# wamuumu/query-recommendation-system

Measured on AMD Instinct MI355X. Metric: MinHash signatures/sec through the whole hot path (signatures -> LSH candidates -> pair scoring -> top-K), higher is better.
Workload: dtype u16/int32 MinHash values, uint64 keys and pairs (integer); float64 cosine

## Files before the change

query-recommendation-system_amd/csrc/pairs.hip:

```cpp
#include "common.h"

constexpr int PAIR_THREADS = 256;
constexpr int PAIR_IPT = 4;
constexpr int PAIR_TILE = PAIR_THREADS * PAIR_IPT;

constexpr int CMP_THREADS = 256;
constexpr int CMP_IPT = 8;
constexpr int CMP_TILE = CMP_THREADS * CMP_IPT;

constexpr int PAIR_HALO = 128;

__device__ static inline uint32_t mix_hi(uint64_t k, int hsh) { return (uint32_t)(qr_mix64(k) >> hsh); }

__device__ static inline void stage_tile(const uint64_t *__restrict__ k, int64_t nq, int64_t tile_start, int hsh,
                                         uint64_t *sk, uint32_t *sh) {
  for (int idx = threadIdx.x; idx < PAIR_HALO + PAIR_TILE; idx += PAIR_THREADS) {
    const int64_t g = tile_start - PAIR_HALO + idx;
    uint64_t key = 0;
    if (g >= 0 && g < nq) key = k[g];
    sk[idx] = key;
    sh[idx] = mix_hi(key, hsh);
  }
}

// ... 845 lines not shown

QRLSH_EXPORT size_t qrlsh_region_unique_workspace_bytes(int64_t nids, int32_t group_bits) {
  if (nids <= 0 || group_bits < 0 || group_bits > 8) return 64;
  const int64_t nr = region_count(nids, group_bits);
  return (size_t)(4 * (nr + 1) + ceil_div64(nr + 1, SCANL_CHUNK) + 2) * sizeof(uint64_t);
}

__global__ __launch_bounds__(256) void region_spans_kernel(const uint32_t *__restrict__ counts, int64_t nr, uint32_t cap,
                                                           uint64_t *__restrict__ starts, uint64_t *__restrict__ ends,
                                                           const uint32_t *__restrict__ scatter_ovf,
                                                           uint64_t *__restrict__ ovf_out) {
  const int64_t r = (int64_t)blockIdx.x * blockDim.x + threadIdx.x;
  if (r == 0 && ovf_out) *ovf_out = *scatter_ovf;
  if (r > nr) return;
  starts[r] = (uint64_t)r * cap;
  ends[r] = (uint64_t)r * cap + (r < nr ? min(counts[r], cap) : 0u);
}

template <typename W = uint64_t>
static int region_unique_count_impl(const char *name, const W *grouped, int64_t n, const uint32_t *regions_counts,
                                    uint32_t cap, int32_t group_bits, int32_t id_bits, int64_t nids, uint64_t *tmp,
                                    void *workspace, size_t workspace_bytes, uint64_t *total_overflow_out, void *stream,
                                    const uint32_t *scatter_ovf = nullptr) {
  QR_CHECK_ARG(n >= 0 && total_overflow_out && nids > 0 && nids <= (1ll << 32), "%s: bad arguments", name);
  QR_CHECK_ARG(group_bits >= 0 && group_bits <= 8 && id_bits >= 1 && id_bits <= 31 && nids <= (1ll << id_bits) &&
                   (group_bits + id_bits < 32 || (group_bits + id_bits == 32 && nids < (1ll << id_bits))),
               "%s: group_bits=%d / id_bits=%d (need group_bits <= 8, id_bits <= 31, group_bits + id_bits <= 32)", name,
               group_bits, id_bits);
  hipStream_t st = static_cast<hipStream_t>(stream);
  if (hipMemsetAsync(total_overflow_out, 0, (scatter_ovf ? 3 : 2) * sizeof(uint64_t), st) != hipSuccess) {
    qrlsh_set_error("%s: hipMemsetAsync failed", name);
    return QRLSH_EHIP;
  }
  if (n == 0) return QRLSH_OK;
  QR_CHECK_ARG(grouped && tmp && workspace, "%s: null pointer", name);
  if (workspace_bytes < qrlsh_region_unique_workspace_bytes(nids, group_bits)) {
    qrlsh_set_error("%s: workspace %zu < %zu bytes", name, workspace_bytes,
                    qrlsh_region_unique_workspace_bytes(nids, group_bits));
    return QRLSH_EWORKSPACE;
  }
  const int64_t nr = region_count(nids, group_bits);
  QR_CHECK_ARG(nr <= 2147483647ll, "%s: too many regions", name);
  uint64_t *starts = static_cast<uint64_t *>(workspace), *counts = starts + (nr + 1), *biglist = counts + (nr + 1);
  uint64_t *nbig = biglist + nr, *sums = nbig + 1;
  uint64_t *ends = sums + ceil_div64(nr + 1, SCANL_CHUNK) + 1;
  if (hipMemsetAsync(counts + nr, 0, sizeof(uint64_t), st) != hipSuccess ||
      hipMemsetAsync(nbig, 0, sizeof(uint64_t), st) != hipSuccess) {
    qrlsh_set_error("%s: hipMemsetAsync failed", name);
    return QRLSH_EHIP;
  }
  if (regions_counts) {
    QR_LAUNCH("region_bounds", region_spans_kernel, dim3((unsigned)ceil_div64(nr + 1, 256)), dim3(256), 0, st, regions_counts,
              nr, cap, starts, ends, scatter_ovf, scatter_ovf ? total_overflow_out + 2 : nullptr);
  } else {
    if constexpr (sizeof(W) == 8) {
      QR_LAUNCH("region_bounds", region_bounds_kernel, dim3((unsigned)ceil_div64(nr + 1, 256)), dim3(256), 0, st, grouped, n,
                32 + group_bits, nr, starts);
    }
    ends = starts + 1;
  }
  QR_LAUNCH("region_unique", region_unique_kernel<W>, dim3((unsigned)nr), dim3(RG_THREADS), 0, st, grouped,
            (const uint64_t *)starts, (const uint64_t *)ends, tmp, counts, biglist,
            reinterpret_cast<unsigned long long *>(nbig), group_bits, id_bits);
  QR_LAUNCH("region_unique_big", region_unique_big_kernel<W>, dim3((unsigned)(nr < RG_BIG_GRID ? nr : RG_BIG_GRID)),
            dim3(RG_THREADS), 0, st, grouped, (const uint64_t *)starts, (const uint64_t *)ends, tmp, counts,
            (const uint64_t *)biglist, (const unsigned long long *)nbig, total_overflow_out + 1, group_bits, id_bits);
  qr_scan_u64(counts, nr + 1, total_overflow_out, sums, st);
  QR_LAUNCH_CHECK(name);
  return QRLSH_OK;
}

QRLSH_EXPORT int qrlsh_region_unique_count(const uint64_t *grouped, int64_t n, int32_t group_bits, int32_t id_bits,
                                           int64_t nids, uint64_t *tmp, void *workspace, size_t workspace_bytes,
                                           uint64_t *total_overflow_out, void *stream) {
  return region_unique_count_impl("qrlsh_region_unique_count", grouped, n, nullptr, 0u, group_bits, id_bits, nids, tmp,
                                  workspace, workspace_bytes, total_overflow_out, stream);
}

QRLSH_EXPORT int qrlsh_region_unique_count_regions(const uint64_t *regions, const uint32_t *counts, int64_t cap, int64_t n,
                                                   int32_t group_bits, int32_t id_bits, int64_t nids, uint64_t *tmp,
                                                   void *workspace, size_t workspace_bytes, uint64_t *total_overflow_out,
                                                   void *stream) {
  QR_CHECK_ARG(counts && cap > 0 && cap < (1ll << 32), "qrlsh_region_unique_count_regions: bad arguments");
  return region_unique_count_impl("qrlsh_region_unique_count_regions", regions, n, counts, (uint32_t)cap, group_bits, id_bits,
                                  nids, tmp, workspace, workspace_bytes, total_overflow_out, stream);
}

QRLSH_EXPORT int qrlsh_region_unique_count_regions3(const uint64_t *regions, const uint32_t *counts, int64_t cap, int64_t n,
                                                    int32_t group_bits, int32_t id_bits, int64_t nids, uint64_t *tmp,
                                                    void *workspace, size_t workspace_bytes, const uint32_t *scatter_overflow,
                                                    uint64_t *out3, void *stream) {
  QR_CHECK_ARG(counts && scatter_overflow && cap > 0 && cap < (1ll << 32), "qrlsh_region_unique_count_regions3: bad arguments");
  return region_unique_count_impl("qrlsh_region_unique_count_regions3", regions, n, counts, (uint32_t)cap, group_bits, id_bits,
                                  nids, tmp, workspace, workspace_bytes, out3, stream, scatter_overflow);
}

QRLSH_EXPORT int qrlsh_region_unique_count_regions32(const uint32_t *regions, const uint32_t *counts, int64_t cap, int64_t n,
                                                     int32_t group_bits, int32_t id_bits, int64_t nids, uint64_t *tmp,
                                                     void *workspace, size_t workspace_bytes,
                                                     const uint32_t *scatter_overflow, uint64_t *out3, void *stream) {
  QR_CHECK_ARG(counts && scatter_overflow && cap > 0 && cap < (1ll << 32), "qrlsh_region_unique_count_regions32: bad arguments");
  return region_unique_count_impl<uint32_t>("qrlsh_region_unique_count_regions32", regions, n, counts, (uint32_t)cap, group_bits,
                                            id_bits, nids, tmp, workspace, workspace_bytes, out3, stream, scatter_overflow);
}

QRLSH_EXPORT int qrlsh_region_unique_fill(const uint64_t *tmp, int64_t n, int32_t group_bits, int64_t nids,
                                          const void *workspace, uint64_t *out, void *stream) {
  QR_CHECK_ARG(n >= 0 && nids > 0 && group_bits >= 0 && group_bits <= 8, "qrlsh_region_unique_fill: bad arguments");
  if (n == 0) return QRLSH_OK;
  QR_CHECK_ARG(tmp && workspace && out, "qrlsh_region_unique_fill: null pointer");
  const int64_t nr = region_count(nids, group_bits);
  const uint64_t *starts = static_cast<const uint64_t *>(workspace), *offs = starts + (nr + 1);
  QR_LAUNCH("region_gather", region_gather_kernel, dim3((unsigned)nr), dim3(256), 0, static_cast<hipStream_t>(stream), tmp,
            offs, starts, out);
  QR_LAUNCH_CHECK("qrlsh_region_unique_fill");
  return QRLSH_OK;
}

QRLSH_EXPORT int qrlsh_topk_count(const uint64_t *sorted_edges, int64_t n_edges, int32_t K, int32_t id_bits,
                                  void *workspace, size_t workspace_bytes, uint64_t *total_out, void *stream) {
  QR_CHECK_ARG(K > 0 && id_bits >= 0 && id_bits <= 32, "qrlsh_topk_count: bad K=%d or id_bits=%d (need <= 32)", K,
               id_bits);
  return compact_count<PRED_TOPK>(sorted_edges, n_edges, K, id_bits + 11, workspace, workspace_bytes, total_out, stream,
                                  "qrlsh_topk_count");
}

QRLSH_EXPORT int qrlsh_topk_fill(const uint64_t *sorted_edges, const uint32_t *sorted_dst, int64_t n_edges, int32_t K,
                                 int32_t id_bits, const void *workspace, int32_t *src_out, int32_t *dst_out,
                                 int32_t *milli_out, void *stream) {
  return qrlsh_topk_fill_based(sorted_edges, sorted_dst, n_edges, K, id_bits, 0, workspace, src_out, dst_out, milli_out,
                               stream);
}

QRLSH_EXPORT int qrlsh_topk_fill_based(const uint64_t *sorted_edges, const uint32_t *sorted_dst, int64_t n_edges,
                                       int32_t K, int32_t id_bits, int64_t src_base, const void *workspace,
                                       int32_t *src_out, int32_t *dst_out, int32_t *milli_out, void *stream) {
  QR_CHECK_ARG(K > 0 && id_bits >= 0 && id_bits <= 32 && n_edges >= 0 && src_base >= 0 && src_base < (1ll << 31),
               "qrlsh_topk_fill: bad arguments");
  QR_CHECK_ARG((id_bits == 0) == (sorted_dst != nullptr), "qrlsh_topk_fill: sorted_dst goes with id_bits == 0");
  if (n_edges == 0) return QRLSH_OK;
  QR_CHECK_ARG(sorted_edges && workspace && src_out && dst_out && milli_out, "qrlsh_topk_fill: null pointer");
  QR_LAUNCH("topk_fill", (compact_fill_kernel<PRED_TOPK>), dim3((unsigned)ceil_div64(n_edges, CMP_TILE)),
                     dim3(CMP_THREADS), 0, static_cast<hipStream_t>(stream), sorted_edges, n_edges, K, id_bits + 11,
                     id_bits, sorted_dst, static_cast<const uint64_t *>(workspace), nullptr, src_out, dst_out, milli_out,
                     (int32_t)src_base);
  QR_LAUNCH_CHECK("qrlsh_topk_fill");
  return QRLSH_OK;
}

__device__ static inline uint32_t rev_src(uint64_t w, int id_bits, bool wide) {
  return (uint32_t)(wide ? w >> 11 : w >> (id_bits + 11));
}

constexpr uint32_t SEL_UNSET = 0xFFFFFFFFu;
constexpr int SEL_GAP = 32;
constexpr int EB_RUN = 4;
__device__ static inline int64_t edge_src(const uint64_t *__restrict__ a, int64_t t, bool fwd, int id_bits, bool wide) {
  return (int64_t)(fwd ? (uint32_t)(a[t] >> 32) : rev_src(a[t], id_bits, wide));
}
__global__ __launch_bounds__(256) void edge_bounds_kernel(const uint64_t *__restrict__ pairs,
                                                          const uint64_t *__restrict__ rev, int64_t n, int64_t nq,
                                                          int id_bits, int wide, uint32_t *__restrict__ fstart,
                                                          uint32_t *__restrict__ rstart, int y0 = 0) {
  const bool fwd = blockIdx.y + y0 == 0;
  const uint64_t *a = fwd ? pairs : rev;
  uint32_t *start = fwd ? fstart : rstart;
  const bool w = wide != 0;
  const int64_t t0 = ((int64_t)blockIdx.x * blockDim.x + threadIdx.x) * EB_RUN;
  uint64_t x[EB_RUN];
  if (t0 + EB_RUN <= n && ((uintptr_t)a & 15) == 0) {
    const ulonglong2 *v = reinterpret_cast<const ulonglong2 *>(a + t0);
#pragma unroll
    for (int k = 0; k < EB_RUN; k += 2) {
      const ulonglong2 u = v[k >> 1];
      x[k] = u.x;
      x[k + 1] = u.y;
    }
  } else {
#pragma unroll
    for (int k = 0; k < EB_RUN; ++k) x[k] = t0 + k < n ? a[t0 + k] : 0ull;
  }
  int64_t s[EB_RUN];
#pragma unroll
  for (int k = 0; k < EB_RUN; ++k)
    s[k] = t0 + k < n ? (int64_t)(fwd ? (uint32_t)(x[k] >> 32) : rev_src(x[k], id_bits, w)) : nq;
  int64_t p = __shfl_up(s[EB_RUN - 1], 1, WAVE);
  if ((threadIdx.x & (WAVE - 1)) == 0) p = t0 > 0 && t0 <= n ? edge_src(a, t0 - 1, fwd, id_bits, w) : -1;
#pragma unroll
  for (int k = 0; k < EB_RUN; ++k) {
    const int64_t t = t0 + k;
    if (t > n) break;
    if (s[k] - p > SEL_GAP) {
      if (s[k] <= nq) start[s[k]] = (uint32_t)t;
    } else {
      for (int64_t q = p + 1; q <= s[k] && q <= nq; ++q) start[q] = (uint32_t)t;
    }
    p = s[k];
  }
}

__global__ __launch_bounds__(256) void edge_bounds_fix_kernel(const uint64_t *__restrict__ pairs,
                                                              const uint64_t *__restrict__ rev, int64_t n, int64_t nq,
                                                              int id_bits, int wide, uint32_t *__restrict__ fstart,
                                                              uint32_t *__restrict__ rstart, int y0 = 0) {
  const bool fwd = blockIdx.y + y0 == 0;
  const uint64_t *a = fwd ? pairs : rev;
  uint32_t *start = fwd ? fstart : rstart;
  const int64_t q = (int64_t)blockIdx.x * blockDim.x + threadIdx.x;
  if (q > nq || start[q] != SEL_UNSET) return;
  int64_t lo = 0, hi = n;
  while (lo < hi) {
    const int64_t mid = (lo + hi) >> 1;
    if (edge_src(a, mid, fwd, id_bits, wide != 0) >= q) hi = mid;
    else lo = mid + 1;
  }
  start[q] = (uint32_t)lo;
}

constexpr int SEL_SHORT = 16;
constexpr int SEL_LONG = 64;
constexpr int SEL_MAXK = 256;
constexpr int SEL_LIST_GRID = 1024;

constexpr int LEN_QPB = 4096;
__global__ __launch_bounds__(256) void topk_len_kernel(const uint32_t *__restrict__ fstart,
                                                       const uint32_t *__restrict__ rstart, int64_t nq, int K,
                                                       uint64_t *__restrict__ cnt, uint32_t *__restrict__ medlist,
                                                       uint32_t *__restrict__ longlist,
                                                       unsigned long long *__restrict__ nlists,
                                                       uint64_t *__restrict__ wgsum) {
  __shared__ uint32_t smed[LEN_QPB], slng[LEN_QPB], sval[LEN_QPB + LEN_QPB / 16];
  __shared__ uint64_t sscan[4];
  __shared__ uint32_t nmed, nlng;
  __shared__ unsigned long long bmed, blng;
  const int lane = threadIdx.x & (WAVE - 1);
  const uint64_t lt_mask = (1ull << lane) - 1ull;
  auto lpad = [](int i) { return i + (i >> 4); };
  if (threadIdx.x == 0) {
    nmed = 0;
    nlng = 0;
  }
  __syncthreads();
  const int64_t q0 = (int64_t)blockIdx.x * LEN_QPB;
#pragma unroll 4
  for (int it = 0; it < LEN_QPB / 256; ++it) {
    const int64_t q = q0 + it * 256 + threadIdx.x;
    uint64_t c = 0;
    if (q < nq) c = (uint64_t)(fstart[q + 1] - fstart[q]) + (rstart[q + 1] - rstart[q]);
    sval[lpad(it * 256 + threadIdx.x)] = (uint32_t)(c > (uint64_t)K ? (uint64_t)K : c);
    const bool med = c > (uint64_t)SEL_SHORT && c <= (uint64_t)SEL_LONG, lng = c > (uint64_t)SEL_LONG;
    const uint64_t mm = __ballot(med), ml = __ballot(lng);
    uint32_t pm = 0, pl = 0;
    if (lane == 0) {
      if (mm) pm = atomicAdd(&nmed, (uint32_t)__popcll(mm));
      if (ml) pl = atomicAdd(&nlng, (uint32_t)__popcll(ml));
    }
    pm = __shfl(pm, 0, WAVE);
    pl = __shfl(pl, 0, WAVE);
    if (med) smed[pm + (uint32_t)__popcll(mm & lt_mask)] = (uint32_t)q;
    if (lng) slng[pl + (uint32_t)__popcll(ml & lt_mask)] = (uint32_t)q;
  }
  __syncthreads();
  if (threadIdx.x == 0) {
    bmed = nmed ? __hip_atomic_fetch_add(&nlists[0], (unsigned long long)nmed, __ATOMIC_RELAXED, __HIP_MEMORY_SCOPE_AGENT) : 0ull;
    blng = nlng ? __hip_atomic_fetch_add(&nlists[1], (unsigned long long)nlng, __ATOMIC_RELAXED, __HIP_MEMORY_SCOPE_AGENT) : 0ull;
  }
  __syncthreads();
  for (uint32_t k = threadIdx.x; k < nmed; k += 256) medlist[bmed + k] = smed[k];
  for (uint32_t k = threadIdx.x; k < nlng; k += 256) longlist[blng + k] = slng[k];
  constexpr int PER = LEN_QPB / 256;
  uint32_t v[PER], sum = 0;
#pragma unroll
  for (int k = 0; k < PER; ++k) {
    v[k] = sval[lpad(threadIdx.x * PER + k)];
    sum += v[k];
  }
  uint64_t total;
  uint32_t run = (uint32_t)block_excl_scan_u64_256((uint64_t)sum, sscan, &total);
#pragma unroll
  for (int k = 0; k < PER; ++k) {
    sval[lpad(threadIdx.x * PER + k)] = run;
    run += v[k];
  }
  __syncthreads();
  for (int k = threadIdx.x; k < LEN_QPB; k += 256)
    if (q0 + k <= nq) cnt[q0 + k] = sval[lpad(k)];
  if (threadIdx.x == 0) wgsum[blockIdx.x] = total;
}

__global__ __launch_bounds__(256) void topk_off_add_kernel(uint64_t *__restrict__ off, int64_t m,
                                                           const uint64_t *__restrict__ wgsum) {
  const uint64_t add = wgsum[blockIdx.x];
  const int64_t q0 = (int64_t)blockIdx.x * LEN_QPB;
  if (add == 0) return;
#pragma unroll 4
  for (int k = threadIdx.x; k < LEN_QPB; k += 256)
    if (q0 + k < m) off[q0 + k] += add;
}

__device__ static inline uint64_t sel_key(uint32_t x, uint32_t rs, uint32_t nr, uint32_t fs,
                                          const uint64_t *__restrict__ pairs, const int32_t *__restrict__ milli,
                                          const uint64_t *__restrict__ rev, const uint32_t *__restrict__ rdst,
                                          int id_bits, uint64_t idm) {
  if (x < nr) {
    const uint64_t w = rev[rs + x];
    return rdst ? (w & 0x7FFull) << 32 | rdst[rs + x] : ((w >> id_bits) & 0x7FFull) << 32 | (w & idm);
  }
  const uint32_t y = fs + (x - nr);
  return (uint64_t)(uint32_t)(1000 - milli[y]) << 32 | (uint32_t)pairs[y];
}

template <int S> __device__ static inline uint64_t row_ror64(uint64_t v) {
  const int lo = __builtin_amdgcn_update_dpp(0, (int)(uint32_t)v, 0x120 + S, 0xF, 0xF, false);
  const int hi = __builtin_amdgcn_update_dpp(0, (int)(uint32_t)(v >> 32), 0x120 + S, 0xF, 0xF, false);
  return (uint64_t)(uint32_t)hi << 32 | (uint32_t)lo;
}
template <int S> __device__ static inline uint32_t row_rank(uint64_t mine) {
  uint32_t r = row_ror64<S>(mine) < mine;
  if constexpr (S > 1) r += row_rank<S - 1>(mine);
  return r;
}

constexpr int SEL_QPG = 4;
__global__ __launch_bounds__(256) void topk_select_short_kernel(const uint64_t *__restrict__ pairs,
                                                                const int32_t *__restrict__ milli,
                                                                const uint64_t *__restrict__ rev,
                                                                const uint32_t *__restrict__ rdst,
                                                                const uint32_t *__restrict__ fstart,
                                                                const uint32_t *__restrict__ rstart,
                                                                const uint64_t *__restrict__ off, int64_t nq, int K,
                                                                int id_bits, int32_t *__restrict__ src_out,
                                                                int32_t *__restrict__ dst_out,
                                                                int32_t *__restrict__ milli_out) {
  const int64_t group = ((int64_t)blockIdx.x * blockDim.x + threadIdx.x) >> 4;
  const int64_t ngroups = ((int64_t)gridDim.x * blockDim.x) >> 4;
  const uint32_t l = threadIdx.x & 15;
  const uint64_t idm = id_bits >= 32 ? 0xFFFFFFFFull : (1ull << id_bits) - 1ull;
  uint32_t fs[SEL_QPG], rs[SEL_QPG], nr[SEL_QPG], len[SEL_QPG];
  uint64_t o0[SEL_QPG], mine[SEL_QPG];
#pragma unroll
  for (int c = 0; c < SEL_QPG; ++c) {
    const int64_t q = group + (int64_t)c * ngroups;
    uint32_t nf = 0;
    fs[c] = rs[c] = nr[c] = 0;
    o0[c] = 0;
    if (q < nq) {
      fs[c] = fstart[q];
      nf = fstart[q + 1] - fs[c];
      rs[c] = rstart[q];
      nr[c] = rstart[q + 1] - rs[c];
      o0[c] = off[q];
    }
    len[c] = nf + nr[c];
    if (len[c] > (uint32_t)SEL_SHORT) len[c] = 0;
  }
#pragma unroll
  for (int c = 0; c < SEL_QPG; ++c)
    mine[c] = l < len[c] ? sel_key(l, rs[c], nr[c], fs[c], pairs, milli, rev, rdst, id_bits, idm) : ~0ull;
#pragma unroll
  for (int c = 0; c < SEL_QPG; ++c) {
    const uint32_t rank = row_rank<15>(mine[c]);
    if (l < len[c] && rank < (uint32_t)K) {
      const uint64_t o = o0[c] + rank;
      src_out[o] = (int32_t)(group + (int64_t)c * ngroups);
      dst_out[o] = (int32_t)(uint32_t)mine[c];
      milli_out[o] = 1000 - (int32_t)(uint32_t)(mine[c] >> 32);
    }
  }
}

__global__ __launch_bounds__(256) void topk_select_medium_kernel(const uint64_t *__restrict__ pairs,
                                                                 const int32_t *__restrict__ milli,
                                                                 const uint64_t *__restrict__ rev,
                                                                 const uint32_t *__restrict__ rdst,
                                                                 const uint32_t *__restrict__ fstart,
                                                                 const uint32_t *__restrict__ rstart,
                                                                 const uint64_t *__restrict__ off,
                                                                 const uint32_t *__restrict__ medlist,
                                                                 const unsigned long long *__restrict__ nlists, int K,
                                                                 int id_bits, int32_t *__restrict__ src_out,
                                                                 int32_t *__restrict__ dst_out,
                                                                 int32_t *__restrict__ milli_out) {
  const int lane = threadIdx.x & (WAVE - 1);
  const uint64_t idm = id_bits >= 32 ? 0xFFFFFFFFull : (1ull << id_bits) - 1ull;
  const unsigned long long nm = nlists[0], nwaves = (unsigned long long)gridDim.x * (blockDim.x / WAVE);
  for (unsigned long long e = (unsigned long long)blockIdx.x * (blockDim.x / WAVE) + (threadIdx.x >> 6); e < nm;
       e += nwaves) {
    const uint32_t q = medlist[e];
    const uint32_t fs = fstart[q], nf = fstart[q + 1] - fs, rs = rstart[q], nr = rstart[q + 1] - rs;
    const uint32_t len = nf + nr;
    const uint64_t mine = (uint32_t)lane < len ? sel_key(lane, rs, nr, fs, pairs, milli, rev, rdst, id_bits, idm) : ~0ull;
    uint32_t rank = 0;
#pragma unroll 9
    for (int s = 1; s < WAVE; ++s) {
      const int from = (lane + s) & (WAVE - 1);
      const uint32_t lo = (uint32_t)__shfl((int)(uint32_t)mine, from, WAVE), hi = (uint32_t)__shfl((int)(uint32_t)(mine >> 32), from, WAVE);
      rank += ((uint64_t)hi << 32 | lo) < mine;
    }
    if ((uint32_t)lane < len && rank < (uint32_t)K) {
      const uint64_t o = off[q] + rank;
      src_out[o] = (int32_t)q;
      dst_out[o] = (int32_t)(uint32_t)mine;
      milli_out[o] = 1000 - (int32_t)(uint32_t)(mine >> 32);
    }
  }
}

__global__ __launch_bounds__(256) void topk_select_long_kernel(const uint64_t *__restrict__ pairs,
                                                               const int32_t *__restrict__ milli,
                                                               const uint64_t *__restrict__ rev,
                                                               const uint32_t *__restrict__ rdst,
                                                               const uint32_t *__restrict__ fstart,
                                                               const uint32_t *__restrict__ rstart,
                                                               const uint64_t *__restrict__ off,
                                                               const uint32_t *__restrict__ longlist,
                                                               const unsigned long long *__restrict__ nlists, int K,
                                                               int id_bits, int32_t *__restrict__ src_out,
                                                               int32_t *__restrict__ dst_out,
                                                               int32_t *__restrict__ milli_out, int by_id) {
  constexpr int NV = 2048;
  __shared__ uint32_t hist_all[4][NV];
  __shared__ uint64_t keep_all[4][SEL_MAXK];
  const int lane = threadIdx.x & (WAVE - 1), wv = threadIdx.x >> 6;
  uint32_t *hist = hist_all[wv];
  uint64_t *keep = keep_all[wv];
  const uint64_t idm = id_bits >= 32 ? 0xFFFFFFFFull : (1ull << id_bits) - 1ull;
  const unsigned long long nl = nlists[1];
  const unsigned long long nwaves = (unsigned long long)gridDim.x * 4;
  const uint64_t lt_mask = (1ull << lane) - 1ull;
  for (unsigned long long e = (unsigned long long)blockIdx.x * 4 + wv; e < nl; e += nwaves) {
    const uint32_t q = longlist[e];
    const uint32_t fs = fstart[q], nf = fstart[q + 1] - fs, rs = rstart[q], nr = rstart[q + 1] - rs;
    const uint32_t len = nf + nr;
    for (int v = lane; v < NV; v += WAVE) hist[v] = 0;
    __builtin_amdgcn_wave_barrier();
    for (uint32_t x = lane; x < len; x += WAVE)
      atomicAdd(&hist[(uint32_t)(sel_key(x, rs, nr, fs, pairs, milli, rev, rdst, id_bits, idm) >> 32)], 1u);
    __builtin_amdgcn_wave_barrier();
    uint32_t mysum = 0;
    for (int v = 0; v < NV / WAVE; ++v) mysum += hist[lane * (NV / WAVE) + v];
    uint32_t inc = mysum;
#pragma unroll
    for (int d = 1; d < WAVE; d <<= 1) {
      const uint32_t o = __shfl_up(inc, d, WAVE);
      if (lane >= d) inc += o;
    }
    const uint64_t reach = __ballot(inc >= (uint32_t)K);
    uint32_t vstar = NV, below = 0;
    if (reach) {
      const int owner = __ffsll((long long)reach) - 1;
      uint32_t run = __shfl(inc - mysum, owner, WAVE);
      uint32_t vs = NV, bl = 0;
      if (lane == owner) {
        for (int v = 0; v < NV / WAVE; ++v) {
          const uint32_t h = hist[lane * (NV / WAVE) + v];
          if (run + h >= (uint32_t)K) {
            vs = lane * (NV / WAVE) + v;
            bl = run;
            break;
          }
          run += h;
        }
      }
      vstar = __shfl(vs, owner, WAVE);
      below = __shfl(bl, owner, WAVE);
    }
    const uint32_t want_eq = reach ? (uint32_t)K - below : 0u;
    uint32_t id_cut = 0xFFFFFFFFu;
    if (by_id && reach && hist[vstar] > want_eq) {
      uint32_t prefix = 0, need = want_eq;
      for (int shift = 22; shift >= 0; shift -= 11) {
        __builtin_amdgcn_wave_barrier();
        for (int v = lane; v < NV; v += WAVE) hist[v] = 0;
        __builtin_amdgcn_wave_barrier();
        for (uint32_t x = lane; x < len; x += WAVE) {
          const uint64_t k = sel_key(x, rs, nr, fs, pairs, milli, rev, rdst, id_bits, idm);
          const uint32_t idv = (uint32_t)k;
          if ((uint32_t)(k >> 32) == vstar && (shift == 22 || (idv >> (shift + 11)) == prefix))
            atomicAdd(&hist[(idv >> shift) & (NV - 1)], 1u);
        }
        __builtin_amdgcn_wave_barrier();
        uint32_t ms = 0;
        for (int v = 0; v < NV / WAVE; ++v) ms += hist[lane * (NV / WAVE) + v];
        uint32_t ic = ms;
#pragma unroll
        for (int d = 1; d < WAVE; d <<= 1) {
          const uint32_t o = __shfl_up(ic, d, WAVE);
          if (lane >= d) ic += o;
        }
        const int owner = __ffsll((long long)__ballot(ic >= need)) - 1;
        uint32_t run = __shfl(ic - ms, owner, WAVE), dg = 0, bl = 0;
        if (lane == owner) {
          for (int v = 0; v < NV / WAVE; ++v) {
            const uint32_t h = hist[lane * (NV / WAVE) + v];
            if (run + h >= need) {
              dg = lane * (NV / WAVE) + v;
              bl = run;
              break;
            }
            run += h;
          }
        }
        dg = __shfl(dg, owner, WAVE);
        bl = __shfl(bl, owner, WAVE);
        prefix = shift == 22 ? dg : (prefix << 11 | dg);
        need -= bl;
      }
      id_cut = prefix;
    }
    uint32_t nkeep = 0, neq = 0;
    for (uint32_t x0 = 0; x0 < len; x0 += WAVE) {
      const uint32_t x = x0 + lane;
      const uint64_t k = x < len ? sel_key(x, rs, nr, fs, pairs, milli, rev, rdst, id_bits, idm) : ~0ull;
      const uint32_t inv = (uint32_t)(k >> 32);
      const bool lt = x < len && inv < vstar;
      const bool eq = x < len && inv == vstar;
      const uint64_t meq = __ballot(eq);
      const bool take_eq = eq && (id_cut != 0xFFFFFFFFu ? (uint32_t)k <= id_cut
                                                        : neq + (uint32_t)__popcll(meq & lt_mask) < want_eq);
      const uint64_t mk = __ballot(lt || take_eq);
      if (lt || take_eq) keep[nkeep + (uint32_t)__popcll(mk & lt_mask)] = k;
      nkeep += (uint32_t)__popcll(mk);
      neq += (uint32_t)__popcll(meq);
    }
    __builtin_amdgcn_wave_barrier();
    const uint64_t o0 = off[q];
    for (uint32_t a = lane; a < nkeep; a += WAVE) {
      const uint64_t k = keep[a];
      uint32_t r = 0;
      for (uint32_t c = 0; c < nkeep; ++c) r += keep[c] < k;
      src_out[o0 + r] = (int32_t)q;
      dst_out[o0 + r] = (int32_t)(uint32_t)k;
      milli_out[o0 + r] = 1000 - (int32_t)(uint32_t)(k >> 32);
    }
    __builtin_amdgcn_wave_barrier();
  }
}

struct SelWs {
  uint32_t *fstart, *rstart, *medlist, *longlist;
  uint64_t *off, *nlong, *sums;
  size_t bytes;
};
static SelWs sel_ws(void *workspace, int64_t nq) {
  SelWs w;
  char *p = static_cast<char *>(workspace);
  size_t o = 0;
  w.fstart = reinterpret_cast<uint32_t *>(p + o);
  o += ((size_t)(nq + 1) * 4 + 15) & ~(size_t)15;
  w.rstart = reinterpret_cast<uint32_t *>(p + o);
  o += ((size_t)(nq + 1) * 4 + 15) & ~(size_t)15;
  w.medlist = reinterpret_cast<uint32_t *>(p + o);
  o += ((size_t)(nq + 1) * 4 + 15) & ~(size_t)15;
  w.longlist = reinterpret_cast<uint32_t *>(p + o);
  o += ((size_t)(nq + 1) * 4 + 15) & ~(size_t)15;
  w.off = reinterpret_cast<uint64_t *>(p + o);
  o += (size_t)(nq + 2) * 8;
  w.nlong = reinterpret_cast<uint64_t *>(p + o);
  o += 16;
  w.sums = reinterpret_cast<uint64_t *>(p + o);
  o += (size_t)(ceil_div64(nq + 1, LEN_QPB) + 2) * 8;
  w.bytes = o;
  return w;
}

QRLSH_EXPORT size_t qrlsh_topk_select_workspace_bytes(int64_t nq) {
  if (nq <= 0) return 64;
  return sel_ws(nullptr, nq).bytes;
}

QRLSH_EXPORT int qrlsh_topk_select_count(const uint64_t *pairs, int64_t n, const uint64_t *rev_sorted,
                                         const uint32_t *rev_dst, int64_t nq, int32_t K, int32_t id_bits, void *workspace,
                                         size_t workspace_bytes, uint64_t *total_out, void *stream) {
  QR_CHECK_ARG(n >= 0 && n < (1ll << 31) && nq > 0 && nq <= (1ll << 32) && K > 0 && K <= SEL_MAXK && id_bits >= 1 &&
                   id_bits <= 32,
               "qrlsh_topk_select_count: bad arguments (n=%lld nq=%lld K=%d (<= %d) id_bits=%d)", (long long)n,
               (long long)nq, K, SEL_MAXK, id_bits);
  QR_CHECK_ARG(rev_dst || id_bits <= 26 || (!pairs && ((uint64_t)(nq - 1) >> (53 - id_bits)) == 0),
               "qrlsh_topk_select_count: packed reverse words need id_bits <= 26 (or, without a forward list, src < 2^(53 - id_bits))");
  QR_CHECK_ARG(total_out && workspace && (n == 0 || rev_sorted), "qrlsh_topk_select_count: null pointer");
  if (workspace_bytes < qrlsh_topk_select_workspace_bytes(nq)) {
    qrlsh_set_error("qrlsh_topk_select_count: workspace %zu < %zu bytes", workspace_bytes,
                    qrlsh_topk_select_workspace_bytes(nq));
    return QRLSH_EWORKSPACE;
  }
  hipStream_t st = static_cast<hipStream_t>(stream);
  const SelWs w = sel_ws(workspace, nq);
  if (hipMemsetAsync(w.nlong, 0, 2 * sizeof(uint64_t), st) != hipSuccess) {
    qrlsh_set_error("qrlsh_topk_select_count: hipMemsetAsync failed");
    return QRLSH_EHIP;
  }
  const dim3 blk(256);
  if (hipMemsetAsync(w.fstart, 0xFF, (size_t)((char *)w.medlist - (char *)w.fstart), st) != hipSuccess) {
    qrlsh_set_error("qrlsh_topk_select_count: hipMemsetAsync failed");
    return QRLSH_EHIP;
  }
  const int lists = pairs ? 2 : 1, y0 = pairs ? 0 : 1;
  if (!pairs && hipMemsetAsync(w.fstart, 0, (size_t)((char *)w.rstart - (char *)w.fstart), st) != hipSuccess) {
    qrlsh_set_error("qrlsh_topk_select_count: hipMemsetAsync failed");
    return QRLSH_EHIP;
  }
  QR_LAUNCH("topk_bounds", edge_bounds_kernel, dim3((unsigned)ceil_div64(n + 1, 256 * EB_RUN), lists), blk, 0, st, pairs,
            rev_sorted, n, nq, id_bits, rev_dst ? 1 : 0, w.fstart, w.rstart, y0);
  QR_LAUNCH("topk_bounds", edge_bounds_fix_kernel, dim3((unsigned)ceil_div64(nq + 1, 256), lists), blk, 0, st, pairs,
            rev_sorted, n, nq, id_bits, rev_dst ? 1 : 0, w.fstart, w.rstart, y0);
  QR_LAUNCH("topk_len", topk_len_kernel, dim3((unsigned)ceil_div64(nq + 1, LEN_QPB)), blk, 0, st, (const uint32_t *)w.fstart,
            (const uint32_t *)w.rstart, nq, K, w.off, w.medlist, w.longlist,
            reinterpret_cast<unsigned long long *>(w.nlong), w.sums);
  const int64_t nwg = ceil_div64(nq + 1, LEN_QPB);
  QR_LAUNCH("scan_blocks", scan_u64_kernel, dim3(1), dim3(1024), 0, st, w.sums, nwg, total_out);
  QR_LAUNCH("scan_blocks", topk_off_add_kernel, dim3((unsigned)nwg), blk, 0, st, w.off, nq + 1, (const uint64_t *)w.sums);
  QR_LAUNCH_CHECK("qrlsh_topk_select_count");
  return QRLSH_OK;
}

QRLSH_EXPORT int qrlsh_topk_select_fill(const uint64_t *pairs, const int32_t *milli, int64_t n,
                                        const uint64_t *rev_sorted, const uint32_t *rev_dst, int64_t nq, int32_t K,
                                        int32_t id_bits, const void *workspace, int32_t *src_out, int32_t *dst_out,
                                        int32_t *milli_out, void *stream) {
  QR_CHECK_ARG(n >= 0 && n < (1ll << 31) && nq > 0 && K > 0 && K <= SEL_MAXK && id_bits >= 1 && id_bits <= 32,
               "qrlsh_topk_select_fill: bad arguments");
  if (n == 0) return QRLSH_OK;
  QR_CHECK_ARG((pairs == nullptr) == (milli == nullptr) && rev_sorted && workspace && src_out && dst_out && milli_out,
               "qrlsh_topk_select_fill: null pointer (pairs and milli: both or neither)");
  const SelWs w = sel_ws(const_cast<void *>(workspace), nq);
  hipStream_t st = static_cast<hipStream_t>(stream);
  const uint32_t *fsp = w.fstart, *rsp = w.rstart;
  const uint64_t *offp = w.off;
  const unsigned long long *nl = reinterpret_cast<const unsigned long long *>(w.nlong);
  QR_LAUNCH("topk_select", topk_select_short_kernel, dim3((unsigned)ceil_div64(nq, 16 * SEL_QPG)), dim3(256), 0, st, pairs, milli,
            rev_sorted, rev_dst, fsp, rsp, offp, nq, K, id_bits, src_out, dst_out, milli_out);
  QR_LAUNCH("topk_select_medium", topk_select_medium_kernel, dim3(SEL_LIST_GRID), dim3(256), 0, st, pairs, milli,
            rev_sorted, rev_dst, fsp, rsp, offp, (const uint32_t *)w.medlist, nl, K, id_bits, src_out, dst_out, milli_out);
  QR_LAUNCH("topk_select_long", topk_select_long_kernel, dim3(SEL_LIST_GRID), dim3(256), 0, st, pairs, milli, rev_sorted,
            rev_dst, fsp, rsp, offp, (const uint32_t *)w.longlist, nl, K, id_bits, src_out, dst_out, milli_out,
            pairs ? 0 : 1);
  QR_LAUNCH_CHECK("qrlsh_topk_select_fill");
  return QRLSH_OK;
}
```

Before: 628.4 million.

## Fuse top-K bounds into tiled kernel and stage short-list selection in LDS

Replaces the memset, edge-bounds and bounds-fix kernels with a per-tile binary search for tile ends plus a fused tile kernel. That kernel marks run starts in shared memory, computes suffix minima to get per-query start offsets, and builds the length lists in the same pass. The short-list selection now stages each block's 256 queries' keys into LDS with coalesced loads instead of gathering per query. The long-list kernel is templated on wide keys and batches its loads. The aim is to cut kernel launches, memsets and scattered global accesses, at the cost of more complex shared-memory logic and some risk on edge cases such as a null pairs array.

```diff
diff --git a/query-recommendation-system_amd/csrc/pairs.hip b/query-recommendation-system_amd/csrc/pairs.hip
--- a/query-recommendation-system_amd/csrc/pairs.hip
+++ b/query-recommendation-system_amd/csrc/pairs.hip
@@ -1021,103 +1021,169 @@
   return (uint32_t)(wide ? w >> 11 : w >> (id_bits + 11));
 }
 
-constexpr uint32_t SEL_UNSET = 0xFFFFFFFFu;
-constexpr int SEL_GAP = 32;
-constexpr int EB_RUN = 4;
 __device__ static inline int64_t edge_src(const uint64_t *__restrict__ a, int64_t t, bool fwd, int id_bits, bool wide) {
   return (int64_t)(fwd ? (uint32_t)(a[t] >> 32) : rev_src(a[t], id_bits, wide));
 }
-__global__ __launch_bounds__(256) void edge_bounds_kernel(const uint64_t *__restrict__ pairs,
-                                                          const uint64_t *__restrict__ rev, int64_t n, int64_t nq,
-                                                          int id_bits, int wide, uint32_t *__restrict__ fstart,
-                                                          uint32_t *__restrict__ rstart, int y0 = 0) {
-  const bool fwd = blockIdx.y + y0 == 0;
+
+constexpr int SEL_SHORT = 16;
+constexpr int SEL_LONG = 64;
+constexpr int SEL_MAXK = 256;
+constexpr int SEL_LIST_GRID = 1024;
+
+constexpr int LEN_QPB = 4096;
+constexpr int LEN_PAD = LEN_QPB + LEN_QPB / 16 + 1;
+constexpr int TILE_RUN = 4;
+__device__ static inline int lpad(int i) { return i + (i >> 4); }
+
+__global__ __launch_bounds__(256) void tile_ends_kernel(const uint64_t *__restrict__ pairs,
+                                                        const uint64_t *__restrict__ rev, int64_t n, int id_bits,
+                                                        int wide, int64_t ntiles, uint32_t *__restrict__ fend,
+                                                        uint32_t *__restrict__ rend) {
+  const int64_t t = (int64_t)blockIdx.x * blockDim.x + threadIdx.x;
+  if (t > ntiles) return;
+  const bool fwd = blockIdx.y == 0;
   const uint64_t *a = fwd ? pairs : rev;
-  uint32_t *start = fwd ? fstart : rstart;
-  const bool w = wide != 0;
-  const int64_t t0 = ((int64_t)blockIdx.x * blockDim.x + threadIdx.x) * EB_RUN;
-  uint64_t x[EB_RUN];
-  if (t0 + EB_RUN <= n && ((uintptr_t)a & 15) == 0) {
-    const ulonglong2 *v = reinterpret_cast<const ulonglong2 *>(a + t0);
-#pragma unroll
-    for (int k = 0; k < EB_RUN; k += 2) {
-      const ulonglong2 u = v[k >> 1];
-      x[k] = u.x;
-      x[k + 1] = u.y;
-    }
-  } else {
-#pragma unroll
-    for (int k = 0; k < EB_RUN; ++k) x[k] = t0 + k < n ? a[t0 + k] : 0ull;
-  }
-  int64_t s[EB_RUN];
-#pragma unroll
-  for (int k = 0; k < EB_RUN; ++k)
-    s[k] = t0 + k < n ? (int64_t)(fwd ? (uint32_t)(x[k] >> 32) : rev_src(x[k], id_bits, w)) : nq;
-  int64_t p = __shfl_up(s[EB_RUN - 1], 1, WAVE);
-  if ((threadIdx.x & (WAVE - 1)) == 0) p = t0 > 0 && t0 <= n ? edge_src(a, t0 - 1, fwd, id_bits, w) : -1;
-#pragma unroll
-  for (int k = 0; k < EB_RUN; ++k) {
-    const int64_t t = t0 + k;
-    if (t > n) break;
-    if (s[k] - p > SEL_GAP) {
-      if (s[k] <= nq) start[s[k]] = (uint32_t)t;
-    } else {
-      for (int64_t q = p + 1; q <= s[k] && q <= nq; ++q) start[q] = (uint32_t)t;
-    }
-    p = s[k];
-  }
-}
-
-__global__ __launch_bounds__(256) void edge_bounds_fix_kernel(const uint64_t *__restrict__ pairs,
-                                                              const uint64_t *__restrict__ rev, int64_t n, int64_t nq,
-                                                              int id_bits, int wide, uint32_t *__restrict__ fstart,
-                                                              uint32_t *__restrict__ rstart, int y0 = 0) {
-  const bool fwd = blockIdx.y + y0 == 0;
-  const uint64_t *a = fwd ? pairs : rev;
-  uint32_t *start = fwd ? fstart : rstart;
-  const int64_t q = (int64_t)blockIdx.x * blockDim.x + threadIdx.x;
-  if (q > nq || start[q] != SEL_UNSET) return;
-  int64_t lo = 0, hi = n;
+  const int64_t q = t * LEN_QPB;
+  int64_t lo = 0, hi = a ? n : 0;
   while (lo < hi) {
     const int64_t mid = (lo + hi) >> 1;
     if (edge_src(a, mid, fwd, id_bits, wide != 0) >= q) hi = mid;
     else lo = mid + 1;
   }
-  start[q] = (uint32_t)lo;
-}
-
-constexpr int SEL_SHORT = 16;
-constexpr int SEL_LONG = 64;
-constexpr int SEL_MAXK = 256;
-constexpr int SEL_LIST_GRID = 1024;
-
-constexpr int LEN_QPB = 4096;
-__global__ __launch_bounds__(256) void topk_len_kernel(const uint32_t *__restrict__ fstart,
-                                                       const uint32_t *__restrict__ rstart, int64_t nq, int K,
-                                                       uint64_t *__restrict__ cnt, uint32_t *__restrict__ medlist,
-                                                       uint32_t *__restrict__ longlist,
-                                                       unsigned long long *__restrict__ nlists,
-                                                       uint64_t *__restrict__ wgsum) {
-  __shared__ uint32_t smed[LEN_QPB], slng[LEN_QPB], sval[LEN_QPB + LEN_QPB / 16];
+  (fwd ? fend : rend)[t] = (uint32_t)lo;
+}
+
+template <bool WHOLE>
+__device__ static inline void tile_mark_step(const uint64_t *__restrict__ a, int64_t base, int64_t b, int64_t e,
+                                             int64_t n, bool fwd, int id_bits, bool wide, int64_t q0, uint32_t *mark) {
+  const int lane = threadIdx.x & (WAVE - 1);
+  uint64_t x[2][TILE_RUN], xp[2];
+#pragma unroll
+  for (int u = 0; u < 2; ++u) {
+    const int64_t t0 = base + (int64_t)(u * 256 + threadIdx.x) * TILE_RUN;
+    if constexpr (WHOLE) {
+      const ulonglong2 *v = reinterpret_cast<const ulonglong2 *>(a + t0);
+#pragma unroll
+      for (int k = 0; k < TILE_RUN; k += 2) {
+        const ulonglong2 w = v[k >> 1];
+        x[u][k] = w.x;
+        x[u][k + 1] = w.y;
+      }
+    } else {
+#pragma unroll
+      for (int k = 0; k < TILE_RUN; ++k) x[u][k] = t0 + k < n ? a[t0 + k] : 0ull;
+    }
+    xp[u] = lane == 0 && t0 > b && t0 < e ? a[t0 - 1] : 0ull;
+  }
+#pragma unroll
+  for (int u = 0; u < 2; ++u) {
+    const int64_t t0 = base + (int64_t)(u * 256 + threadIdx.x) * TILE_RUN;
+    uint32_t s[TILE_RUN];
+#pragma unroll
+    for (int k = 0; k < TILE_RUN; ++k) s[k] = fwd ? (uint32_t)(x[u][k] >> 32) : rev_src(x[u][k], id_bits, wide);
+    uint32_t p = __shfl_up(s[TILE_RUN - 1], 1, WAVE);
+    if (lane == 0) p = fwd ? (uint32_t)(xp[u] >> 32) : rev_src(xp[u], id_bits, wide);
+#pragma unroll
+    for (int k = 0; k < TILE_RUN; ++k) {
+      const int64_t t = t0 + k;
+      const int64_t d = (int64_t)s[k] - q0;
+      if (t >= b && t < e && (t == b || s[k] != p) && d >= 0 && d < LEN_QPB) mark[lpad((int)d)] = (uint32_t)t;
+      p = s[k];
+    }
+  }
+}
+__device__ static inline void tile_mark(const uint64_t *__restrict__ a, int64_t b, int64_t e, int64_t n, bool fwd,
+                                        int id_bits, bool wide, int64_t q0, uint32_t *mark) {
+  const bool al = ((uintptr_t)a & 15) == 0;
+  for (int64_t base = b & ~(int64_t)(TILE_RUN - 1); base < e; base += 2 * 256 * TILE_RUN) {
+    if (al && base + 2 * 256 * TILE_RUN <= n) tile_mark_step<true>(a, base, b, e, n, fwd, id_bits, wide, q0, mark);
+    else tile_mark_step<false>(a, base, b, e, n, fwd, id_bits, wide, q0, mark);
+  }
+}
+
+__device__ static inline void tile_suffix_min(uint32_t *mark, uint32_t end, uint32_t *swave) {
+  constexpr int PER = LEN_QPB / 256;
+  const int lane = threadIdx.x & (WAVE - 1), w = threadIdx.x >> 6;
+  uint32_t v[PER], suf = end;
+#pragma unroll
+  for (int k = 0; k < PER; ++k) {
+    v[k] = mark[lpad(threadIdx.x * PER + k)];
+    suf = v[k] < suf ? v[k] : suf;
+  }
+#pragma unroll
+  for (int d = 1; d < WAVE; d <<= 1) {
+    const uint32_t o = __shfl_down(suf, d, WAVE);
+    if (lane + d < WAVE && o < suf) suf = o;
+  }
+  if (lane == 0) swave[w] = suf;
+  __syncthreads();
+  uint32_t run = end;
+#pragma unroll
+  for (int i = 1; i < 256 / WAVE; ++i)
+    if (i > w && swave[i] < run) run = swave[i];
+  const uint32_t nx = __shfl_down(suf, 1, WAVE);
+  if (lane < WAVE - 1 && nx < run) run = nx;
+#pragma unroll
+  for (int k = PER - 1; k >= 0; --k) {
+    run = v[k] < run ? v[k] : run;
+    mark[lpad(threadIdx.x * PER + k)] = run;
+  }
+  __syncthreads();
+}
+
+__global__ __launch_bounds__(256) void topk_tile_kernel(const uint64_t *__restrict__ pairs,
+                                                        const uint64_t *__restrict__ rev, int64_t n, int64_t nq, int K,
+                                                        int id_bits, int wide, const uint32_t *__restrict__ fend,
+                                                        const uint32_t *__restrict__ rend,
+                                                        uint32_t *__restrict__ fstart, uint32_t *__restrict__ rstart,
+                                                        uint64_t *__restrict__ cnt, uint32_t *__restrict__ medlist,
+                                                        uint32_t *__restrict__ longlist,
+                                                        unsigned long long *__restrict__ nlists,
+                                                        uint64_t *__restrict__ wgsum) {
+  __shared__ uint32_t sf[LEN_PAD], sr[LEN_PAD], sval[LEN_PAD];
+  uint32_t *smed = sf, *slng = sr;
   __shared__ uint64_t sscan[4];
+  __shared__ uint32_t swave[256 / WAVE];
   __shared__ uint32_t nmed, nlng;
   __shared__ unsigned long long bmed, blng;
   const int lane = threadIdx.x & (WAVE - 1);
   const uint64_t lt_mask = (1ull << lane) - 1ull;
-  auto lpad = [](int i) { return i + (i >> 4); };
+  const int64_t q0 = (int64_t)blockIdx.x * LEN_QPB;
+  const uint32_t fb = fend[blockIdx.x], fe = fend[blockIdx.x + 1], rb = rend[blockIdx.x], re = rend[blockIdx.x + 1];
+  for (int k = threadIdx.x; k <= LEN_QPB; k += 256) {
+    sf[lpad(k)] = fe;
+    sr[lpad(k)] = re;
+  }
   if (threadIdx.x == 0) {
     nmed = 0;
     nlng = 0;
   }
   __syncthreads();
-  const int64_t q0 = (int64_t)blockIdx.x * LEN_QPB;
+  if (fb < fe) tile_mark(pairs, fb, fe, n, true, id_bits, false, q0, sf);
+  if (rb < re) tile_mark(rev, rb, re, n, false, id_bits, wide != 0, q0, sr);
+  __syncthreads();
+  tile_suffix_min(sf, fe, swave);
+  tile_suffix_min(sr, re, swave);
+#pragma unroll 4
+  for (int it = 0; it < LEN_QPB / 256; ++it) {
+    const int k = it * 256 + threadIdx.x;
+    const int64_t q = q0 + k;
+    const uint32_t f0 = sf[lpad(k)], r0 = sr[lpad(k)];
+    uint32_t c = 0;
+    if (q < nq) c = (sf[lpad(k + 1)] - f0) + (sr[lpad(k + 1)] - r0);
+    if (q <= nq) {
+      fstart[q] = f0;
+      rstart[q] = r0;
+    }
+    sval[lpad(k)] = c;
+  }
+  __syncthreads();
 #pragma unroll 4
   for (int it = 0; it < LEN_QPB / 256; ++it) {
     const int64_t q = q0 + it * 256 + threadIdx.x;
-    uint64_t c = 0;
-    if (q < nq) c = (uint64_t)(fstart[q + 1] - fstart[q]) + (rstart[q + 1] - rstart[q]);
-    sval[lpad(it * 256 + threadIdx.x)] = (uint32_t)(c > (uint64_t)K ? (uint64_t)K : c);
-    const bool med = c > (uint64_t)SEL_SHORT && c <= (uint64_t)SEL_LONG, lng = c > (uint64_t)SEL_LONG;
+    const uint32_t c = sval[lpad(it * 256 + threadIdx.x)];
+    sval[lpad(it * 256 + threadIdx.x)] = c > (uint32_t)K ? (uint32_t)K : c;
+    const bool med = c > (uint32_t)SEL_SHORT && c <= (uint32_t)SEL_LONG, lng = c > (uint32_t)SEL_LONG;
     const uint64_t mm = __ballot(med), ml = __ballot(lng);
     uint32_t pm = 0, pl = 0;
     if (lane == 0) {
@@ -1190,50 +1256,102 @@
   return r;
 }
 
-constexpr int SEL_QPG = 4;
-__global__ __launch_bounds__(256) void topk_select_short_kernel(const uint64_t *__restrict__ pairs,
-                                                                const int32_t *__restrict__ milli,
-                                                                const uint64_t *__restrict__ rev,
-                                                                const uint32_t *__restrict__ rdst,
-                                                                const uint32_t *__restrict__ fstart,
-                                                                const uint32_t *__restrict__ rstart,
-                                                                const uint64_t *__restrict__ off, int64_t nq, int K,
-                                                                int id_bits, int32_t *__restrict__ src_out,
-                                                                int32_t *__restrict__ dst_out,
-                                                                int32_t *__restrict__ milli_out) {
-  const int64_t group = ((int64_t)blockIdx.x * blockDim.x + threadIdx.x) >> 4;
-  const int64_t ngroups = ((int64_t)gridDim.x * blockDim.x) >> 4;
-  const uint32_t l = threadIdx.x & 15;
+constexpr int SEL_QS = 256;
+constexpr int SEL_STAGE = 4;
+template <bool WIDE>
+__device__ static inline void sel_stage_rev(const uint64_t *__restrict__ rev, const uint32_t *__restrict__ rdst,
+                                            uint32_t rb, uint32_t re, int64_t q0, int id_bits, uint64_t idm,
+                                            const uint32_t *slen, const uint32_t *srb, uint64_t *skey) {
+  for (uint32_t p0 = rb + threadIdx.x; p0 < re + threadIdx.x; p0 += SEL_STAGE * 256) {
+    uint64_t w[SEL_STAGE];
+    uint32_t d[SEL_STAGE];
+#pragma unroll
+    for (int u = 0; u < SEL_STAGE; ++u) {
+      const uint32_t p = p0 + u * 256 < re ? p0 + u * 256 : re - 1;
+      w[u] = rev[p];
+      d[u] = WIDE ? rdst[p] : 0u;
+    }
+#pragma unroll
+    for (int u = 0; u < SEL_STAGE; ++u) {
+      const uint32_t p = p0 + u * 256;
+      const uint32_t ql = (uint32_t)((int64_t)(WIDE ? w[u] >> 11 : w[u] >> (id_bits + 11)) - q0);
+      const uint64_t key = WIDE ? (w[u] & 0x7FFull) << 32 | d[u] : ((w[u] >> id_bits) & 0x7FFull) << 32 | (w[u] & idm);
+      if (p < re && ql < (uint32_t)SEL_QS && slen[ql]) skey[srb[ql] + p] = key;
+    }
+  }
+}
+
+__global__ __launch_bounds__(256) void topk_select_tile_kernel(const uint64_t *__restrict__ pairs,
+                                                               const int32_t *__restrict__ milli,
+                                                               const uint64_t *__restrict__ rev,
+                                                               const uint32_t *__restrict__ rdst,
+                                                               const uint32_t *__restrict__ fstart,
+                                                               const uint32_t *__restrict__ rstart,
+                                                               const uint64_t *__restrict__ off, int64_t nq, int K,
+                                                               int id_bits, int32_t *__restrict__ src_out,
+                                                               int32_t *__restrict__ dst_out,
+                                                               int32_t *__restrict__ milli_out) {
+  __shared__ uint64_t skey[SEL_QS * SEL_SHORT];
+  __shared__ uint64_t sout[SEL_QS], sscan[4];
+  __shared__ uint32_t soff[SEL_QS], slen[SEL_QS], srb[SEL_QS], sfb[SEL_QS], sends[4];
+  const int t = threadIdx.x;
+  const int64_t q0 = (int64_t)blockIdx.x * SEL_QS;
   const uint64_t idm = id_bits >= 32 ? 0xFFFFFFFFull : (1ull << id_bits) - 1ull;
-  uint32_t fs[SEL_QPG], rs[SEL_QPG], nr[SEL_QPG], len[SEL_QPG];
-  uint64_t o0[SEL_QPG], mine[SEL_QPG];
-#pragma unroll
-  for (int c = 0; c < SEL_QPG; ++c) {
-    const int64_t q = group + (int64_t)c * ngroups;
-    uint32_t nf = 0;
-    fs[c] = rs[c] = nr[c] = 0;
-    o0[c] = 0;
-    if (q < nq) {
-      fs[c] = fstart[q];
-      nf = fstart[q + 1] - fs[c];
-      rs[c] = rstart[q];
-      nr[c] = rstart[q + 1] - rs[c];
-      o0[c] = off[q];
-    }
-    len[c] = nf + nr[c];
-    if (len[c] > (uint32_t)SEL_SHORT) len[c] = 0;
-  }
-#pragma unroll
-  for (int c = 0; c < SEL_QPG; ++c)
-    mine[c] = l < len[c] ? sel_key(l, rs[c], nr[c], fs[c], pairs, milli, rev, rdst, id_bits, idm) : ~0ull;
-#pragma unroll
-  for (int c = 0; c < SEL_QPG; ++c) {
-    const uint32_t rank = row_rank<15>(mine[c]);
-    if (l < len[c] && rank < (uint32_t)K) {
-      const uint64_t o = o0[c] + rank;
-      src_out[o] = (int32_t)(group + (int64_t)c * ngroups);
-      dst_out[o] = (int32_t)(uint32_t)mine[c];
-      milli_out[o] = 1000 - (int32_t)(uint32_t)(mine[c] >> 32);
+  {
+    const int64_t qa = q0 + t < nq ? q0 + t : nq, qb = q0 + t + 1 < nq ? q0 + t + 1 : nq;
+    const uint32_t f0 = fstart[qa], f1 = fstart[qb], r0 = rstart[qa], r1 = rstart[qb];
+    const uint32_t nr = r1 - r0, len = nr + (f1 - f0);
+    const uint32_t sl = len <= (uint32_t)SEL_SHORT ? len : 0u;
+    sout[t] = off[qa];
+    uint64_t total;
+    const uint32_t so = (uint32_t)block_excl_scan_u64_256((uint64_t)sl, sscan, &total);
+    soff[t] = so;
+    slen[t] = sl;
+    srb[t] = so - r0;
+    sfb[t] = so + nr - f0;
+    if (t == 0) {
+      sends[0] = r0;
+      sends[1] = f0;
+    }
+    if (t == SEL_QS - 1) {
+      sends[2] = r1;
+      sends[3] = f1;
+    }
+    __syncthreads();
+    if (total == 0) return;
+  }
+  const uint32_t rb = sends[0], fb = sends[1], re = sends[2], fe = sends[3];
+  if (rdst) sel_stage_rev<true>(rev, rdst, rb, re, q0, id_bits, idm, slen, srb, skey);
+  else sel_stage_rev<false>(rev, rdst, rb, re, q0, id_bits, idm, slen, srb, skey);
+  for (uint32_t p0 = fb + t; p0 < fe + t; p0 += SEL_STAGE * 256) {
+    uint64_t w[SEL_STAGE];
+    int32_t m[SEL_STAGE];
+#pragma unroll
+    for (int u = 0; u < SEL_STAGE; ++u) {
+      const uint32_t p = p0 + u * 256 < fe ? p0 + u * 256 : fe - 1;
+      w[u] = pairs[p];
+      m[u] = milli[p];
+    }
+#pragma unroll
+    for (int u = 0; u < SEL_STAGE; ++u) {
+      const uint32_t p = p0 + u * 256;
+      const uint32_t ql = (uint32_t)((int64_t)(w[u] >> 32) - q0);
+      if (p < fe && ql < (uint32_t)SEL_QS && slen[ql])
+        skey[sfb[ql] + p] = (uint64_t)(uint32_t)(1000 - m[u]) << 32 | (uint32_t)w[u];
+    }
+  }
+  __syncthreads();
+  const uint32_t l = t & 15, g = t >> 4;
+#pragma unroll 4
+  for (int it = 0; it < SEL_QS / 16; ++it) {
+    const uint32_t ql = it * 16 + g, sl = slen[ql];
+    const uint64_t mine = l < sl ? skey[soff[ql] + l] : ~0ull;
+    const uint32_t rank = row_rank<15>(mine);
+    if (l < sl && rank < (uint32_t)K) {
+      const uint64_t o = sout[ql] + rank;
+      src_out[o] = (int32_t)(q0 + ql);
+      dst_out[o] = (int32_t)(uint32_t)mine;
+      milli_out[o] = 1000 - (int32_t)(uint32_t)(mine >> 32);
     }
   }
 }
@@ -1275,6 +1393,8 @@
   }
 }
 
+constexpr int SEL_FLY = 4;
+template <bool WIDE>
 __global__ __launch_bounds__(256) void topk_select_long_kernel(const uint64_t *__restrict__ pairs,
                                                                const int32_t *__restrict__ milli,
                                                                const uint64_t *__restrict__ rev,
@@ -1303,8 +1423,22 @@
     const uint32_t len = nf + nr;
     for (int v = lane; v < NV; v += WAVE) hist[v] = 0;
     __builtin_amdgcn_wave_barrier();
-    for (uint32_t x = lane; x < len; x += WAVE)
-      atomicAdd(&hist[(uint32_t)(sel_key(x, rs, nr, fs, pairs, milli, rev, rdst, id_bits, idm) >> 32)], 1u);
+    for (uint32_t x0 = lane; x0 < nr + lane; x0 += SEL_FLY * WAVE) {
+      uint64_t w[SEL_FLY];
+#pragma unroll
+      for (int u = 0; u < SEL_FLY; ++u) w[u] = rev[rs + (x0 + u * WAVE < nr ? x0 + u * WAVE : nr - 1)];
+#pragma unroll
+      for (int u = 0; u < SEL_FLY; ++u)
+        if (x0 + u * WAVE < nr) atomicAdd(&hist[(uint32_t)(WIDE ? w[u] & 0x7FFull : (w[u] >> id_bits) & 0x7FFull)], 1u);
+    }
+    for (uint32_t x0 = lane; x0 < nf + lane; x0 += SEL_FLY * WAVE) {
+      int32_t m[SEL_FLY];
+#pragma unroll
+      for (int u = 0; u < SEL_FLY; ++u) m[u] = milli[fs + (x0 + u * WAVE < nf ? x0 + u * WAVE : nf - 1)];
+#pragma unroll
+      for (int u = 0; u < SEL_FLY; ++u)
+        if (x0 + u * WAVE < nf) atomicAdd(&hist[(uint32_t)(1000 - m[u])], 1u);
+    }
     __builtin_amdgcn_wave_barrier();
     uint32_t mysum = 0;
     for (int v = 0; v < NV / WAVE; ++v) mysum += hist[lane * (NV / WAVE) + v];
@@ -1378,12 +1512,10 @@
       id_cut = prefix;
     }
     uint32_t nkeep = 0, neq = 0;
-    for (uint32_t x0 = 0; x0 < len; x0 += WAVE) {
-      const uint32_t x = x0 + lane;
-      const uint64_t k = x < len ? sel_key(x, rs, nr, fs, pairs, milli, rev, rdst, id_bits, idm) : ~0ull;
+    auto take = [&](uint64_t k, bool in) {
       const uint32_t inv = (uint32_t)(k >> 32);
-      const bool lt = x < len && inv < vstar;
-      const bool eq = x < len && inv == vstar;
+      const bool lt = in && inv < vstar;
+      const bool eq = in && inv == vstar;
       const uint64_t meq = __ballot(eq);
       const bool take_eq = eq && (id_cut != 0xFFFFFFFFu ? (uint32_t)k <= id_cut
                                                         : neq + (uint32_t)__popcll(meq & lt_mask) < want_eq);
@@ -1391,6 +1523,34 @@
       if (lt || take_eq) keep[nkeep + (uint32_t)__popcll(mk & lt_mask)] = k;
       nkeep += (uint32_t)__popcll(mk);
       neq += (uint32_t)__popcll(meq);
+    };
+    for (uint32_t x0 = lane; x0 < nr + lane; x0 += SEL_FLY * WAVE) {
+      uint64_t w[SEL_FLY];
+      uint32_t d[SEL_FLY];
+#pragma unroll
+      for (int u = 0; u < SEL_FLY; ++u) {
+        const uint32_t x = x0 + u * WAVE < nr ? x0 + u * WAVE : nr - 1;
+        w[u] = rev[rs + x];
+        d[u] = WIDE ? rdst[rs + x] : 0u;
+      }
+#pragma unroll
+      for (int u = 0; u < SEL_FLY; ++u)
+        if (x0 - lane + u * WAVE < nr)
+          take(WIDE ? (w[u] & 0x7FFull) << 32 | d[u] : ((w[u] >> id_bits) & 0x7FFull) << 32 | (w[u] & idm),
+               x0 + u * WAVE < nr);
+    }
+    for (uint32_t x0 = lane; x0 < nf + lane; x0 += SEL_FLY * WAVE) {
+      uint64_t w[SEL_FLY];
+      int32_t m[SEL_FLY];
+#pragma unroll
+      for (int u = 0; u < SEL_FLY; ++u) {
+        const uint32_t x = x0 + u * WAVE < nf ? x0 + u * WAVE : nf - 1;
+        w[u] = pairs[fs + x];
+        m[u] = milli[fs + x];
+      }
+#pragma unroll
+      for (int u = 0; u < SEL_FLY; ++u)
+        if (x0 - lane + u * WAVE < nf) take((uint64_t)(uint32_t)(1000 - m[u]) << 32 | (uint32_t)w[u], x0 + u * WAVE < nf);
     }
     __builtin_amdgcn_wave_barrier();
     const uint64_t o0 = off[q];
@@ -1407,7 +1567,7 @@
 }
 
 struct SelWs {
-  uint32_t *fstart, *rstart, *medlist, *longlist;
+  uint32_t *fstart, *rstart, *medlist, *longlist, *fend, *rend;
   uint64_t *off, *nlong, *sums;
   size_t bytes;
 };
@@ -1429,6 +1589,10 @@
   o += 16;
   w.sums = reinterpret_cast<uint64_t *>(p + o);
   o += (size_t)(ceil_div64(nq + 1, LEN_QPB) + 2) * 8;
+  w.fend = reinterpret_cast<uint32_t *>(p + o);
+  o += (size_t)(ceil_div64(nq + 1, LEN_QPB) + 2) * 4;
+  w.rend = reinterpret_cast<uint32_t *>(p + o);
+  o += (size_t)(ceil_div64(nq + 1, LEN_QPB) + 2) * 4;
   w.bytes = o;
   return w;
 }
@@ -1460,23 +1624,12 @@
     return QRLSH_EHIP;
   }
   const dim3 blk(256);
-  if (hipMemsetAsync(w.fstart, 0xFF, (size_t)((char *)w.medlist - (char *)w.fstart), st) != hipSuccess) {
-    qrlsh_set_error("qrlsh_topk_select_count: hipMemsetAsync failed");
-    return QRLSH_EHIP;
-  }
-  const int lists = pairs ? 2 : 1, y0 = pairs ? 0 : 1;
-  if (!pairs && hipMemsetAsync(w.fstart, 0, (size_t)((char *)w.rstart - (char *)w.fstart), st) != hipSuccess) {
-    qrlsh_set_error("qrlsh_topk_select_count: hipMemsetAsync failed");
-    return QRLSH_EHIP;
-  }
-  QR_LAUNCH("topk_bounds", edge_bounds_kernel, dim3((unsigned)ceil_div64(n + 1, 256 * EB_RUN), lists), blk, 0, st, pairs,
-            rev_sorted, n, nq, id_bits, rev_dst ? 1 : 0, w.fstart, w.rstart, y0);
-  QR_LAUNCH("topk_bounds", edge_bounds_fix_kernel, dim3((unsigned)ceil_div64(nq + 1, 256), lists), blk, 0, st, pairs,
-            rev_sorted, n, nq, id_bits, rev_dst ? 1 : 0, w.fstart, w.rstart, y0);
-  QR_LAUNCH("topk_len", topk_len_kernel, dim3((unsigned)ceil_div64(nq + 1, LEN_QPB)), blk, 0, st, (const uint32_t *)w.fstart,
-            (const uint32_t *)w.rstart, nq, K, w.off, w.medlist, w.longlist,
-            reinterpret_cast<unsigned long long *>(w.nlong), w.sums);
   const int64_t nwg = ceil_div64(nq + 1, LEN_QPB);
+  QR_LAUNCH("topk_bounds", tile_ends_kernel, dim3((unsigned)ceil_div64(nwg + 1, 256), 2), blk, 0, st, pairs, rev_sorted, n,
+            id_bits, rev_dst ? 1 : 0, nwg, w.fend, w.rend);
+  QR_LAUNCH("topk_len", topk_tile_kernel, dim3((unsigned)nwg), blk, 0, st, pairs, rev_sorted, n, nq, K, id_bits,
+            rev_dst ? 1 : 0, (const uint32_t *)w.fend, (const uint32_t *)w.rend, w.fstart, w.rstart, w.off, w.medlist,
+            w.longlist, reinterpret_cast<unsigned long long *>(w.nlong), w.sums);
   QR_LAUNCH("scan_blocks", scan_u64_kernel, dim3(1), dim3(1024), 0, st, w.sums, nwg, total_out);
   QR_LAUNCH("scan_blocks", topk_off_add_kernel, dim3((unsigned)nwg), blk, 0, st, w.off, nq + 1, (const uint64_t *)w.sums);
   QR_LAUNCH_CHECK("qrlsh_topk_select_count");
@@ -1497,13 +1650,18 @@
   const uint32_t *fsp = w.fstart, *rsp = w.rstart;
   const uint64_t *offp = w.off;
   const unsigned long long *nl = reinterpret_cast<const unsigned long long *>(w.nlong);
-  QR_LAUNCH("topk_select", topk_select_short_kernel, dim3((unsigned)ceil_div64(nq, 16 * SEL_QPG)), dim3(256), 0, st, pairs, milli,
+  QR_LAUNCH("topk_select", topk_select_tile_kernel, dim3((unsigned)ceil_div64(nq, SEL_QS)), dim3(256), 0, st, pairs, milli,
             rev_sorted, rev_dst, fsp, rsp, offp, nq, K, id_bits, src_out, dst_out, milli_out);
   QR_LAUNCH("topk_select_medium", topk_select_medium_kernel, dim3(SEL_LIST_GRID), dim3(256), 0, st, pairs, milli,
             rev_sorted, rev_dst, fsp, rsp, offp, (const uint32_t *)w.medlist, nl, K, id_bits, src_out, dst_out, milli_out);
-  QR_LAUNCH("topk_select_long", topk_select_long_kernel, dim3(SEL_LIST_GRID), dim3(256), 0, st, pairs, milli, rev_sorted,
-            rev_dst, fsp, rsp, offp, (const uint32_t *)w.longlist, nl, K, id_bits, src_out, dst_out, milli_out,
-            pairs ? 0 : 1);
+  if (rev_dst)
+    QR_LAUNCH("topk_select_long", topk_select_long_kernel<true>, dim3(SEL_LIST_GRID), dim3(256), 0, st, pairs, milli,
+              rev_sorted, rev_dst, fsp, rsp, offp, (const uint32_t *)w.longlist, nl, K, id_bits, src_out, dst_out,
+              milli_out, pairs ? 0 : 1);
+  else
+    QR_LAUNCH("topk_select_long", topk_select_long_kernel<false>, dim3(SEL_LIST_GRID), dim3(256), 0, st, pairs, milli,
+              rev_sorted, rev_dst, fsp, rsp, offp, (const uint32_t *)w.longlist, nl, K, id_bits, src_out, dst_out,
+              milli_out, pairs ? 0 : 1);
   QR_LAUNCH_CHECK("qrlsh_topk_select_fill");
   return QRLSH_OK;
 }
```

Result: faster. 644.9 million (median of 6 runs) (+2.6%).
